# subramen/distributed-pytorch

Hardware: AMD Instinct MI355X
Metric: samples/sec (whole node), toy Linear DDP (higher is better)
Workload: dtype fp32; 1 GPU; model=Linear(20,1), global_batch=32, in_features=20, dataset_size=2048, parallelism=dp1, comm=none, engine=persistent, loss=mse, epoch_block=16

## Files before the change

mi355x_ddp/ops/csrc/toy_kernels.hip:

```cpp

#include <hip/hip_runtime.h>

#include <atomic>
#include <cstdint>
#include <cstdlib>
#include <string>
#include <type_traits>

#include "kernel_common.h"
#include "ops.h"
#include "p2p_mesh.h"

namespace mi355x {


__device__ __forceinline__ bool toy_mfma_db(int K) { return (K & 15) != 0; }

__device__ __forceinline__ float toy_db_wave_sum(const float* dy_s, int B,
                                                 int lane) {
  float dbp = 0.f;
  for (int i = lane; i < B; i += 64) dbp += dy_s[i];
  return wave_sum(dbp);
}

template <int MT, int KT>
__device__ __forceinline__ float toy_tile_step(
    const float* xs, const float* ts, const float* ws, float* dy_s,
    float bterm, bool mfma_db, int B, int K, int use_mse, int r, int q,
    f32x4 (&gacc)[KT]) {
  const float inv2B = 2.f / (float)B;
  float loss_acc = 0.f;
  {
    f32x4 acc[MT];
#pragma unroll
    for (int tm = 0; tm < MT; ++tm) acc[tm] = {0.f, 0.f, 0.f, 0.f};
    for (int k0 = 0; k0 < K; k0 += 4) {
      const int k = k0 + q;
      const float b = (r == 0 && k < K) ? ws[k] : 0.f;
#pragma unroll
      for (int tm = 0; tm < MT; ++tm) {
        const int m = tm * 16 + r;
        const float a = (m < B && k < K) ? xs[m * K + k] : 0.f;
        acc[tm] = __builtin_amdgcn_mfma_f32_16x16x4f32(a, b, acc[tm], 0, 0, 0);
      }
    }
#pragma unroll
    for (int tm = 0; tm < MT; ++tm) {
      if (r == 0) {
#pragma unroll
        for (int i = 0; i < 4; ++i) {
          const int row = tm * 16 + q * 4 + i;
          if (row < B) {
            const float y = acc[tm][i] + bterm;
            float dy;
            if (use_mse) {
              const float d = y - ts[row];
              loss_acc += d * d;
              dy = d * inv2B;
            } else {
              dy = 0.f;
            }
            dy_s[row] = dy;
          }
        }
      }
    }
  }
  __syncthreads();

#pragma unroll
  for (int tk = 0; tk < KT; ++tk) gacc[tk] = {0.f, 0.f, 0.f, 0.f};
  for (int i0 = 0; i0 < B; i0 += 4) {
    const int i = i0 + q;
    const float a = (r == 0 && i < B) ? dy_s[i] : 0.f;
#pragma unroll
    for (int tk = 0; tk < KT; ++tk) {
      const int k = tk * 16 + r;
      const float b = (i < B && k < K) ? xs[i * K + k]
                     : (i < B && k == K && mfma_db) ? 1.f : 0.f;
      gacc[tk] = __builtin_amdgcn_mfma_f32_16x16x4f32(a, b, gacc[tk], 0, 0, 0);
    }
  }
  return loss_acc;
}

template <typename T, int MT, int KT>
__global__ void k_toy_fused(const T* __restrict__ X, const T* __restrict__ Tg,
                            T* __restrict__ param, T* __restrict__ grad,
                            float* __restrict__ loss_out,
                            int B, int K, int use_mse,
                            int w_off, int b_off, float lr) {
  const int lane = threadIdx.x;
  const int r = lane & 15, q = lane >> 4;
  __shared__ float xs[128 * 32];
  __shared__ float ts[128];
  __shared__ float ws[33];
  __shared__ float dy_s[128];

  {
    const int total = B * K;
    for (int i = lane; i < total; i += 64) xs[i] = ldf(&X[i]);
    for (int i = lane; i < B; i += 64) ts[i] = ldf(&Tg[i]);
    if (lane < K) ws[lane] = ldf(&param[w_off + lane]);
    if (lane == K) ws[32] = ldf(&param[b_off]);
  }
  __syncthreads();

  const float bterm = ws[32];
  const bool mfma_db = toy_mfma_db(K);
  f32x4 acc[KT];
  float loss_acc = toy_tile_step<MT, KT>(xs, ts, ws, dy_s, bterm, mfma_db, B,
                                         K, use_mse, r, q, acc);
#pragma unroll
  for (int tk = 0; tk < KT; ++tk) {
    const int k = tk * 16 + r;
    if (q == 0 && k < K) {
      if (lr > 0.f) stf(&param[w_off + k], ws[k] - lr * acc[tk][0]);
      else stf(&grad[w_off + k], acc[tk][0]);
    } else if (q == 0 && k == K && mfma_db) {
      if (lr > 0.f) stf(&param[b_off], bterm - lr * acc[tk][0]);
      else stf(&grad[b_off], acc[tk][0]);
    }
  }
  if (!mfma_db) {
    const float dbp = toy_db_wave_sum(dy_s, B, lane);
    if (lane == 0) {
      if (lr > 0.f) stf(&param[b_off], bterm - lr * dbp);
      else stf(&grad[b_off], dbp);
    }
  }
  if (use_mse && loss_out) loss_acc = wave_sum(loss_acc);
  if (lane == 0 && loss_out) *loss_out = use_mse ? loss_acc / (float)B : 0.f;
}

template <typename T>
__device__ __forceinline__ float round_store(float v);
template <>
__device__ __forceinline__ float round_store<float>(float v) { return v; }
template <>
__device__ __forceinline__ float round_store<__hip_bfloat16>(float v) {
  return __bfloat162float(__float2bfloat16(v));
}

template <typename T, int MT, int KT>
__global__ void k_toy_multistep(const T* __restrict__ X,
                                const T* __restrict__ Tg,
                                T* __restrict__ param,
                                float* __restrict__ loss_out,
                                int B, int K, int S, int use_mse,
                                int w_off, int b_off, float lr) {
  constexpr int NR = (MT * 16 * KT * 16 + 63) / 64;
  constexpr int NT = (MT * 16 + 63) / 64;
  const int lane = threadIdx.x;
  const int r = lane & 15, q = lane >> 4;
  __shared__ float xs2[2][128 * 32];
  __shared__ float ts2[2][128];
  __shared__ float ws[33];
  __shared__ float dy_s[128];

  if (lane < K) ws[lane] = ldf(&param[w_off + lane]);
  if (lane == K) ws[32] = ldf(&param[b_off]);

  const int total = B * K;
  float xr[NR], tr[NT];
#pragma unroll
  for (int j = 0; j < NR; ++j) {
    const int i = lane + j * 64;
    if (i < total) xr[j] = ldf(&X[i]);
  }
#pragma unroll
  for (int j = 0; j < NT; ++j) {
    const int i = lane + j * 64;
    if (i < B) tr[j] = ldf(&Tg[i]);
  }

  float loss_last = 0.f;
  for (int s = 0; s < S; ++s) {
    const int buf = s & 1;
    float* xs = xs2[buf];
    float* ts = ts2[buf];
#pragma unroll
    for (int j = 0; j < NR; ++j) {
      const int i = lane + j * 64;
      if (i < total) xs[i] = xr[j];
    }
#pragma unroll
    for (int j = 0; j < NT; ++j) {
      const int i = lane + j * 64;
      if (i < B) ts[i] = tr[j];
    }
    __syncthreads();
    if (s + 1 < S) {
      const T* Xn = X + (size_t)(s + 1) * total;
      const T* Tn = Tg + (size_t)(s + 1) * B;
#pragma unroll
      for (int j = 0; j < NR; ++j) {
        const int i = lane + j * 64;
        if (i < total) xr[j] = ldf(&Xn[i]);
      }
#pragma unroll
      for (int j = 0; j < NT; ++j) {
        const int i = lane + j * 64;
        if (i < B) tr[j] = ldf(&Tn[i]);
      }
    }

    const float bterm = ws[32];
    const bool mfma_db = toy_mfma_db(K);
    f32x4 acc[KT];
    const float loss_acc = toy_tile_step<MT, KT>(
        xs, ts, ws, dy_s, bterm, mfma_db, B, K, use_mse, r, q, acc);
    __syncthreads();
#pragma unroll
    for (int tk = 0; tk < KT; ++tk) {
      const int k = tk * 16 + r;
      if (q == 0 && k < K)
        ws[k] = round_store<T>(ws[k] - lr * acc[tk][0]);
      else if (q == 0 && k == K && mfma_db)
        ws[32] = round_store<T>(bterm - lr * acc[tk][0]);
    }
    if (!mfma_db) {
      const float dbp = toy_db_wave_sum(dy_s, B, lane);
      if (lane == 0) ws[32] = round_store<T>(bterm - lr * dbp);
    }
    if (use_mse && loss_out && s == S - 1) loss_last = wave_sum(loss_acc);
    __syncthreads();
  }

  if (lane < K) stf(&param[w_off + lane], ws[lane]);
  if (lane == K) stf(&param[b_off], ws[32]);
  if (lane == 0 && loss_out) *loss_out = use_mse ? loss_last / (float)B : 0.f;
}

struct MeshArgs {
  MeshSlot* const* peer_slots = nullptr;
  MeshSlot* my_mb = nullptr;
  int world = 1;
  float inv_world = 1.f;
  unsigned long long seq0 = 0;
  unsigned int* err = nullptr;
};

template <int KT>
__device__ __forceinline__ bool mesh_exchange(float (&gval)[KT], int K_,
                                              int lane, int r, int q,
                                              const MeshArgs& m, int s) {
  const unsigned long long sq = m.seq0 + (unsigned long long)s;
  if (q == 0) {
#pragma unroll
    for (int tk = 0; tk < KT; ++tk) {
      const int k = tk * 16 + r;
      if (k <= K_) {
        for (int p = 0; p < m.world; ++p) m.peer_slots[p]->data[k] = gval[tk];
      }
    }
  }
  __threadfence_system();
  __syncthreads();
  if (lane == 0) {
    for (int p = 0; p < m.world; ++p)
      __hip_atomic_store(&m.peer_slots[p]->seq, sq, __ATOMIC_RELEASE,
                         __HIP_MEMORY_SCOPE_SYSTEM);
  }
  bool timed_out = false;
  if (lane < m.world) {
    const unsigned long long t0c = __builtin_amdgcn_s_memrealtime();
    while (__hip_atomic_load(&m.my_mb[lane].seq, __ATOMIC_ACQUIRE,
                             __HIP_MEMORY_SCOPE_SYSTEM) < sq) {
      if (__builtin_amdgcn_s_memrealtime() - t0c > 500000000ull) {
        timed_out = true;
        break;
      }
      __builtin_amdgcn_s_sleep(8);
    }
  }
  if (__any(timed_out)) return false;
  __threadfence_system();
  __syncthreads();
  if (q == 0) {
#pragma unroll
    for (int tk = 0; tk < KT; ++tk) {
      const int k = tk * 16 + r;
      if (k <= K_) {
        float sum = 0.f;
        for (int p = 0; p < m.world; ++p) sum += m.my_mb[p].data[k];
        gval[tk] = sum * m.inv_world;
      }
    }
  }
  return true;
}

template <int B_, int K_, bool MESH = false>
__global__ void __launch_bounds__(64, 1)
k_toy_multistep_spec(const float* __restrict__ X, const float* __restrict__ Tg,
                     float* __restrict__ param, float* __restrict__ loss_out,
                     int S, int use_mse, int w_off, int b_off, float lr,
                     MeshSlot* const* __restrict__ peer_slots,
                     MeshSlot* __restrict__ my_mb, int mworld,
                     float minv_world, unsigned long long seq0,
                     unsigned int* __restrict__ mesh_err) {
  static_assert(B_ % 16 == 0, "whole 16-row tiles: rows carry no guards");
  constexpr int MT = B_ / 16;
  constexpr int KT = (K_ + 15) / 16;
  constexpr int KS = (K_ + 3) / 4;
  constexpr int BS = B_ / 4;
  const int lane = threadIdx.x;
  const int r = lane & 15, q = lane >> 4;
  __shared__ float ws[33];
  __shared__ float dy_s[B_];

  if (lane < K_) ws[lane] = param[w_off + lane];
  if (lane == K_) ws[32] = param[b_off];
  const float inv2B = 2.f / (float)B_;
  float wreg[KT];
#pragma unroll
  for (int tk = 0; tk < KT; ++tk) {
    const int k = tk * 16 + r;
    wreg[tk] = (k < K_) ? param[w_off + ((k < K_) ? k : 0)] : 0.f;
  }

  float cfA[MT][KS];
  float cbB[KT][BS];
  float ctR[MT][4];

  auto prefetch = [&](int s) {
    const float* Xs = X + (size_t)s * (B_ * K_);
    const float* Ts = Tg + (size_t)s * B_;
#pragma unroll
    for (int tm = 0; tm < MT; ++tm) {
      const int m = tm * 16 + r;
#pragma unroll
      for (int kk = 0; kk < KS; ++kk) {
        const int k = 4 * kk + q;
        const int kc = (k < K_) ? k : K_ - 1;
        cfA[tm][kk] = Xs[m * K_ + kc];
      }
    }
#pragma unroll
    for (int tk = 0; tk < KT; ++tk) {
      const int k = tk * 16 + r;
      const int kc = (k < K_) ? k : K_ - 1;
#pragma unroll
      for (int ii = 0; ii < BS; ++ii) cbB[tk][ii] = Xs[(4 * ii + q) * K_ + kc];
    }
#pragma unroll
    for (int tm = 0; tm < MT; ++tm)
#pragma unroll
      for (int i = 0; i < 4; ++i) ctR[tm][i] = Ts[tm * 16 + q * 4 + i];
  };

  prefetch(0);
  float loss_last = 0.f;
  for (int s = 0; s < S; ++s) {
    float wv[KS];
#pragma unroll
    for (int kk = 0; kk < KS; ++kk) {
      const int k = 4 * kk + q;
      const float v = ws[(k < K_) ? k : K_ - 1];
      wv[kk] = (r == 0 && k < K_) ? v : 0.f;
    }
    const float bterm = ws[32];

    f32x4 acc[MT];
#pragma unroll
    for (int tm = 0; tm < MT; ++tm) acc[tm] = {0.f, 0.f, 0.f, 0.f};
#pragma unroll
    for (int kk = 0; kk < KS; ++kk)
#pragma unroll
      for (int tm = 0; tm < MT; ++tm)
        acc[tm] = __builtin_amdgcn_mfma_f32_16x16x4f32(cfA[tm][kk], wv[kk],
                                                       acc[tm], 0, 0, 0);

    float loss_acc = 0.f;
    if (r == 0) {
#pragma unroll
      for (int tm = 0; tm < MT; ++tm)
#pragma unroll
        for (int i = 0; i < 4; ++i) {
          float dy = 0.f;
          if (use_mse) {
            const float d = acc[tm][i] + bterm - ctR[tm][i];
            loss_acc = __builtin_fmaf(d, d, loss_acc);
            dy = d * inv2B;
          }
          dy_s[tm * 16 + q * 4 + i] = dy;
        }
    }
    __syncthreads();

    float av[BS];
#pragma unroll
    for (int ii = 0; ii < BS; ++ii) {
      const float v = dy_s[4 * ii + q];
      av[ii] = (r == 0) ? v : 0.f;
    }
    f32x4 gacc[KT];
#pragma unroll
    for (int tk = 0; tk < KT; ++tk) gacc[tk] = {0.f, 0.f, 0.f, 0.f};
    static_assert(K_ % 16 != 0, "free db column requires K_ % 16 != 0");
#pragma unroll
    for (int ii = 0; ii < BS; ++ii)
#pragma unroll
      for (int tk = 0; tk < KT; ++tk) {
        const int k = tk * 16 + r;
        const float bop = (k == K_) ? 1.f : cbB[tk][ii];
        gacc[tk] = __builtin_amdgcn_mfma_f32_16x16x4f32(av[ii], bop,
                                                        gacc[tk], 0, 0, 0);
      }

    if (s + 1 < S) prefetch(s + 1);

    if (use_mse && loss_out && s == S - 1) loss_last = wave_sum(loss_acc);

    if constexpr (MESH) {
      float gval[KT];
#pragma unroll
      for (int tk = 0; tk < KT; ++tk) gval[tk] = gacc[tk][0];
      const MeshArgs m{peer_slots, my_mb, mworld, minv_world, seq0, mesh_err};
      if (!mesh_exchange<KT>(gval, K_, lane, r, q, m, s)) {
        if (lane == 0) *mesh_err = 1u;
        return;
      }
#pragma unroll
      for (int tk = 0; tk < KT; ++tk) gacc[tk][0] = gval[tk];
    }

#pragma unroll
    for (int tk = 0; tk < KT; ++tk) {
      const int k = tk * 16 + r;
      if (q == 0 && k < K_) {
        wreg[tk] = wreg[tk] - lr * gacc[tk][0];
        ws[k] = wreg[tk];
      } else if (q == 0 && k == K_) {
        ws[32] = bterm - lr * gacc[tk][0];
      }
    }
    __syncthreads();
  }

  if (lane < K_) param[w_off + lane] = ws[lane];
  if (lane == K_) param[b_off] = ws[32];
  if (lane == 0 && loss_out) *loss_out = use_mse ? loss_last / (float)B_ : 0.f;
}

template <int B_, int K_, bool MESH = false>
__global__ void __launch_bounds__(64, 1)
k_toy_multistep_bf16w(const __hip_bfloat16* __restrict__ X,
                      const __hip_bfloat16* __restrict__ Tg,
                      __hip_bfloat16* __restrict__ param,
                      float* __restrict__ loss_out,
                      int S, int use_mse, int w_off, int b_off, float lr,
                      MeshSlot* const* __restrict__ peer_slots,
                      MeshSlot* __restrict__ my_mb, int mworld,
                      float minv_world, unsigned long long seq0,
                      unsigned int* __restrict__ mesh_err) {
  static_assert((B_ == 32 || B_ == 64) && K_ <= 32,
                "bf16 wide path: B in {32, 64}, K<=32");
  constexpr int MT = B_ / 16;
  constexpr int BT = B_ / 32;
  constexpr int KT = (K_ + 15) / 16;
  const int lane = threadIdx.x;
  const int r = lane & 15, q = lane >> 4;
  __shared__ float ws[33];
  __shared__ float dy_s[B_];

  if (lane < K_) ws[lane] = ldf(&param[w_off + lane]);
  if (lane == K_) ws[32] = ldf(&param[b_off]);
  const float inv2B = 2.f / (float)B_;
  float wreg[KT];
#pragma unroll
  for (int tk = 0; tk < KT; ++tk) {
    const int k = tk * 16 + r;
    wreg[tk] = (k < K_) ? ldf(&param[w_off + ((k < K_) ? k : 0)]) : 0.f;
  }

  struct BSet {
    bf16x8 fa[MT];
    bf16x8 bb[BT][KT];
    float tR[MT][4];
  };
  BSet setA, setB;

  auto prefetch = [&](BSet& R, int s) {
    const __hip_bfloat16* Xs = X + (size_t)s * (B_ * K_);
    const __hip_bfloat16* Ts = Tg + (size_t)s * B_;
#pragma unroll
    for (int tm = 0; tm < MT; ++tm) {
      const int m = tm * 16 + r;
#pragma unroll
      for (int j = 0; j < 8; ++j) {
        const int k = q * 8 + j;
        const int kc = (k < K_) ? k : K_ - 1;
        R.fa[tm][j] = *reinterpret_cast<const __bf16*>(&Xs[(size_t)m * K_ + kc]);
      }
    }
#pragma unroll
    for (int bt = 0; bt < BT; ++bt)
#pragma unroll
      for (int tk = 0; tk < KT; ++tk) {
        const int k = tk * 16 + r;
        const int kc = (k < K_) ? k : K_ - 1;
#pragma unroll
        for (int j = 0; j < 8; ++j) {
          const int i = bt * 32 + q * 8 + j;
          R.bb[bt][tk][j] =
              *reinterpret_cast<const __bf16*>(&Xs[(size_t)i * K_ + kc]);
        }
      }
#pragma unroll
    for (int tm = 0; tm < MT; ++tm)
#pragma unroll
      for (int i = 0; i < 4; ++i)
        R.tR[tm][i] = ldf(&Ts[tm * 16 + q * 4 + i]);
  };

  prefetch(setA, 0);
  if (S > 1) prefetch(setB, 1);
  float loss_last = 0.f;
  auto body = [&](BSet& R, int s) {
    const bf16x8* cfa = R.fa;
    const auto& cbb = R.bb;
    const auto& ctR = R.tR;
    bf16x8 b8{};
#pragma unroll
    for (int j = 0; j < 8; ++j) {
      const int k = q * 8 + j;
      const float v = ws[(k < K_) ? k : K_ - 1];
      b8[j] = (r == 0 && k < K_) ? (__bf16)v : (__bf16)0.f;
    }
    const float bterm = ws[32];

    f32x4 acc[MT];
#pragma unroll
    for (int tm = 0; tm < MT; ++tm) {
      acc[tm] = {0.f, 0.f, 0.f, 0.f};
      acc[tm] = __builtin_amdgcn_mfma_f32_16x16x32_bf16(cfa[tm], b8,
                                                        acc[tm], 0, 0, 0);
    }

    float loss_acc = 0.f;
    if (r == 0) {
#pragma unroll
      for (int tm = 0; tm < MT; ++tm)
#pragma unroll
        for (int i = 0; i < 4; ++i) {
          const int row = tm * 16 + q * 4 + i;
          float dy = 0.f;
          if (use_mse) {
            const float d = acc[tm][i] + bterm - ctR[tm][i];
            loss_acc += d * d;
            dy = d * inv2B;
          }
          dy_s[row] = dy;
        }
    }
    __syncthreads();

    bf16x8 a8[BT];
#pragma unroll
    for (int bt = 0; bt < BT; ++bt)
#pragma unroll
      for (int j = 0; j < 8; ++j) {
        const float v = dy_s[bt * 32 + q * 8 + j];
        a8[bt][j] = (r == 0) ? (__bf16)v : (__bf16)0.f;
      }
    f32x4 gacc[KT];
    static_assert(K_ % 16 != 0, "free db column requires K_ % 16 != 0");
#pragma unroll
    for (int tk = 0; tk < KT; ++tk) {
      gacc[tk] = {0.f, 0.f, 0.f, 0.f};
#pragma unroll
      for (int bt = 0; bt < BT; ++bt) {
        bf16x8 bb = cbb[bt][tk];
        if (tk * 16 + r == K_) {
#pragma unroll
          for (int j = 0; j < 8; ++j) bb[j] = (__bf16)1.f;
        }
        gacc[tk] = __builtin_amdgcn_mfma_f32_16x16x32_bf16(a8[bt], bb,
                                                           gacc[tk], 0, 0, 0);
      }
    }

    if (s + 2 < S) prefetch(R, s + 2);

    if (use_mse && loss_out && s == S - 1) loss_last = wave_sum(loss_acc);

    if constexpr (MESH) {
      float gval[KT];
#pragma unroll
      for (int tk = 0; tk < KT; ++tk) gval[tk] = gacc[tk][0];
      const MeshArgs m{peer_slots, my_mb, mworld, minv_world, seq0, mesh_err};
      if (!mesh_exchange<KT>(gval, K_, lane, r, q, m, s)) {
        if (lane == 0) *mesh_err = 1u;
        return false;
      }
#pragma unroll
      for (int tk = 0; tk < KT; ++tk) gacc[tk][0] = gval[tk];
    }

#pragma unroll
    for (int tk = 0; tk < KT; ++tk) {
      const int k = tk * 16 + r;
      if (q == 0 && k < K_) {
        wreg[tk] = round_store<__hip_bfloat16>(wreg[tk] - lr * gacc[tk][0]);
        ws[k] = wreg[tk];
      } else if (q == 0 && k == K_) {
        ws[32] = round_store<__hip_bfloat16>(bterm - lr * gacc[tk][0]);
      }
    }
    __syncthreads();
    return true;
  };

  int s = 0;
  for (; s + 2 <= S; s += 2) {
    if (!body(setA, s)) return;
    if (!body(setB, s + 1)) return;
  }
  if (s < S && !body(setA, s)) return;

  if (lane < K_) stf(&param[w_off + lane], ws[lane]);
  if (lane == K_) stf(&param[b_off], ws[32]);
  if (lane == 0 && loss_out) *loss_out = use_mse ? loss_last / (float)B_ : 0.f;
}


struct RowPair {
  float lo, hi;
};
__device__ __forceinline__ RowPair bcast_rows01(float v, float v2) {
  const auto r = __builtin_amdgcn_permlane16_swap(
      __float_as_uint(v), __float_as_uint(v2), false, false);
  return {__uint_as_float(r[0]), __uint_as_float(r[1])};
}
__device__ __forceinline__ RowPair bcast_rows01(float v) {
  return bcast_rows01(v, v);
}
__device__ __forceinline__ RowPair bcast_halves(float v, float v2) {
  const auto r = __builtin_amdgcn_permlane32_swap(
      __float_as_uint(v), __float_as_uint(v2), false, false);
  return {__uint_as_float(r[0]), __uint_as_float(r[1])};
}
__device__ __forceinline__ RowPair bcast_halves(float v) {
  return bcast_halves(v, v);
}

#define BC_DPP(n) " row_newbcast:" #n " row_mask:0xf bank_mask:0xf\n\t"
#define BC_FMAC(src, x, n) \
  "v_fmac_f32_dpp %[acc], %[" #src "], %[" #x "]" BC_DPP(n)
#define BC_FMAC4(src, p, n0, n1, n2, n3)                  \
  BC_FMAC(src, p##0, n0) BC_FMAC(src, p##1, n1)           \
  BC_FMAC(src, p##2, n2) BC_FMAC(src, p##3, n3)
#define BC_FMAC16(src, p)                                             \
  BC_FMAC4(src, p##0, 0, 1, 2, 3) BC_FMAC4(src, p##1, 4, 5, 6, 7)     \
  BC_FMAC4(src, p##2, 8, 9, 10, 11) BC_FMAC4(src, p##3, 12, 13, 14, 15)
#define BC_IN4(p, x)                                            \
  [p##0] "v"((x)[0]), [p##1] "v"((x)[1]), [p##2] "v"((x)[2]),   \
  [p##3] "v"((x)[3])
#define BC_IN16(p, x)                                     \
  BC_IN4(p##0, (x)) , BC_IN4(p##1, (x) + 4),              \
  BC_IN4(p##2, (x) + 8), BC_IN4(p##3, (x) + 12)
#define BC_PAD "s_nop 1\n\t"
#define BC_ZERO "v_mov_b32 %[acc], 0\n\ts_nop 0\n\t"


template <bool MSE>
__device__ __forceinline__ void chain_fwd20(const RowPair& w,
                                            const float (&x)[20], float t,
                                            float scale, float& d,
                                            float& dy) {
  float acc;
  if constexpr (MSE) {
    asm volatile(BC_ZERO BC_FMAC16(lo, a) BC_FMAC4(hi, b, 0, 1, 2, 3)
                 "v_add_f32_dpp %[acc], %[hi], %[acc]" BC_DPP(4)
                 "v_sub_f32 %[d], %[acc], %[t]\n\t"
                 "v_mul_f32 %[dy], %[c], %[d]"
                 : [acc] "=&v"(acc), [d] "=&v"(d), [dy] "=&v"(dy)
                 : [lo] "v"(w.lo), [hi] "v"(w.hi), BC_IN16(a, x),
                   BC_IN4(b, x + 16), [t] "v"(t), [c] "s"(scale)
                 : "memory");
  } else {
    asm volatile(BC_ZERO BC_FMAC16(lo, a) BC_FMAC4(hi, b, 0, 1, 2, 3)
                 "v_add_f32_dpp %[acc], %[hi], %[acc]" BC_DPP(4)
                 "v_sub_f32 %[d], %[acc], %[t]"
                 : [acc] "=&v"(acc), [d] "=&v"(d)
                 : [lo] "v"(w.lo), [hi] "v"(w.hi), BC_IN16(a, x),
                   BC_IN4(b, x + 16), [t] "v"(t)
                 : "memory");
    dy = 0.f;
  }
}
enum ChainLink { kStart, kPad, kPlain };
template <ChainLink LINK>
__device__ __forceinline__ void chain_bwd16(float& acc, float src,
                                            const float* x) {
  if constexpr (LINK == kStart)
    asm volatile(BC_ZERO BC_FMAC16(s, a)
                 : [acc] "=&v"(acc)
                 : [s] "v"(src), BC_IN16(a, x));
  else if constexpr (LINK == kPad)
    asm volatile(BC_PAD BC_FMAC16(s, a)
                 : [acc] "+v"(acc)
                 : [s] "v"(src), BC_IN16(a, x));
  else
    asm volatile(BC_FMAC16(s, a)
                 : [acc] "+v"(acc)
                 : [s] "v"(src), BC_IN16(a, x));
}
__device__ __forceinline__ void chain_bwd16_update(float& acc, float src,
                                                   const float* x, float& w,
                                                   float lr) {
  asm volatile(BC_FMAC16(s, a) "v_fma_f32 %[w], -%[lr], %[acc], %[w]"
               : [acc] "+v"(acc), [w] "+v"(w)
               : [s] "v"(src), BC_IN16(a, x), [lr] "s"(lr));
}
#undef BC_ZERO
#undef BC_PAD
#undef BC_IN16
#undef BC_IN4
#undef BC_FMAC16
#undef BC_FMAC4
#undef BC_FMAC
#undef BC_DPP

template <int B_, int K_>
struct ChainSlot {
  static constexpr int kPitch = B_ + 4;
  static constexpr int kRow = 0;
  static constexpr int kTr = B_ * K_;
  static constexpr int kOnes = kTr + K_ * kPitch;
  static constexpr int kTgt = kTr + (K_ + 1) * kPitch;
  static constexpr int kSize = kTgt + B_;
  static constexpr int kMaxH = (64 * 1024 / 4) / kSize / 2;
  static_assert(kSize % 4 == 0 && kTr % 4 == 0 && kPitch % 4 == 0 &&
                    K_ % 4 == 0 && B_ % 4 == 0,
                "every ds_read_b128 must be 16-byte aligned");
};

static constexpr int kChainTilesAhead = 4;

template <int B_, int K_, int NL>
__global__ void __launch_bounds__(64 * (1 + NL))
k_toy_multistep_chain(const float* __restrict__ X,
                      const float* __restrict__ Tg,
                      float* __restrict__ param, float* __restrict__ loss_out,
                      int S, int H, int use_mse, int w_off, int b_off,
                      float lr) {
  static_assert((B_ == 32 || B_ == 64) && K_ == 20 && NL >= 1 && NL <= 3,
                "chain path: B in {32, 64}, K = 20, one wave per SIMD");
  using L = ChainSlot<B_, K_>;
  __shared__ __attribute__((aligned(16))) float ring[2 * L::kMaxH * L::kSize];
  const int wave = __builtin_amdgcn_readfirstlane((int)(threadIdx.x >> 6));

  if (wave != 0) {
    constexpr int NT = 64 * NL;
    constexpr int NX = (B_ * K_ + NT - 1) / NT;
    constexpr bool kTail = (B_ * K_) % NT != 0;
    constexpr int R = kChainTilesAhead;
    const int lt = (int)threadIdx.x - 64;
    const int total = (S + H - 1) / H * H;
    float xv[R][NX], tv[R];

    auto load_tile = [&](float (&x)[NX], float& t, int tile) {
      const int tc = tile < S ? tile : S - 1;
      const float* xt = X + (size_t)tc * (B_ * K_);
#pragma unroll
      for (int i = 0; i < NX; ++i) {
        const int f = lt + i * NT;
        x[i] = xt[(kTail && i == NX - 1 && f >= B_ * K_) ? B_ * K_ - 1 : f];
      }
      t = Tg[(size_t)tc * B_ + (lt & (B_ - 1))];
    };
    auto write_tile = [&](const float (&x)[NX], float t, int slot) {
      float* sl = ring + slot * L::kSize;
#pragma unroll
      for (int i = 0; i < NX; ++i) {
        const int f = lt + i * NT;
        if (!kTail || i < NX - 1 || f < B_ * K_) {
          sl[L::kRow + f] = x[i];
          sl[L::kTr + (f % K_) * L::kPitch + f / K_] = x[i];
        }
      }
      if (lt < B_) sl[L::kTgt + lt] = t;
    };

#pragma unroll
    for (int r = 0; r < R; ++r) load_tile(xv[r], tv[r], r);
    if (lt < B_)
      for (int sl = 0; sl < 2 * H; ++sl) ring[sl * L::kSize + L::kOnes + lt] = 1.f;
    int slot = 0, togo = H;
    for (int t0 = 0; t0 < total; t0 += R) {
#pragma unroll
      for (int r = 0; r < R; ++r) {
        const int tile = t0 + r;
        if (tile < S) write_tile(xv[r], tv[r], slot);
        load_tile(xv[r], tv[r], tile + R);
        slot = (slot + 1 == 2 * H) ? 0 : slot + 1;
        if (--togo == 0) {
          togo = H;
          if (tile < total) __syncthreads();
        }
      }
    }
    return;
  }

  const int lane = threadIdx.x;
  const int mr = lane & (B_ - 1);
  const int cr = (lane <= K_) ? lane : (lane & 15);
  const float inv2B = 2.f / (float)B_;
  float wv = param[(lane < K_) ? w_off + lane : b_off];
  const float* rowp = ring + L::kRow + mr * K_;
  const float* colp = ring + L::kTr + cr * L::kPitch;
  const float* tgtp = ring + L::kTgt + mr;

  struct LSet {
    f32x4 xr[K_ / 4];
    f32x4 xc[B_ / 4];
    float t;
  };
  LSet setA, setB;

  auto fetch = [&](LSet& R, int o) {
#pragma unroll
    for (int j = 0; j < K_ / 4; ++j)
      R.xr[j] = *reinterpret_cast<const f32x4*>(rowp + o + 4 * j);
#pragma unroll
    for (int j = 0; j < B_ / 4; ++j)
      R.xc[j] = *reinterpret_cast<const f32x4*>(colp + o + 4 * j);
    R.t = tgtp[o];
  };
  auto settle = [&](LSet& R) {
    static_assert(K_ == 20, "five row reads");
    if constexpr (B_ == 64)
      asm volatile(""
                   : "+v"(R.xc[8]), "+v"(R.xc[9]), "+v"(R.xc[10]),
                     "+v"(R.xc[11]), "+v"(R.xc[12]), "+v"(R.xc[13]),
                     "+v"(R.xc[14]), "+v"(R.xc[15]));
    asm volatile(""
                 : "+v"(R.xr[0]), "+v"(R.xr[1]), "+v"(R.xr[2]), "+v"(R.xr[3]),
                   "+v"(R.xr[4]), "+v"(R.xc[0]), "+v"(R.xc[1]), "+v"(R.xc[2]),
                   "+v"(R.xc[3]), "+v"(R.xc[4]), "+v"(R.xc[5]), "+v"(R.xc[6]),
                   "+v"(R.xc[7]), "+v"(R.t)
                 :
                 : "memory");
  };

  struct CSet {
    float xr[K_];
    float xc[B_];
    float t;
  };
  float wa, wb;
  auto dup = [&] {
    wa = wv, wb = wv;
    asm volatile("" : "+v"(wa), "+v"(wb)::"memory");
  };
  float d_last = 0.f;
  auto compute = [&](const LSet& V, auto mse) {
    CSet R;
#pragma unroll
    for (int k = 0; k < K_; ++k) R.xr[k] = V.xr[k / 4][k % 4];
#pragma unroll
    for (int i = 0; i < B_; ++i) R.xc[i] = V.xc[i / 4][i % 4];
    R.t = V.t;
    RowPair w;
    if constexpr (B_ == 64) w = bcast_rows01(bcast_halves(wa, wb).lo);
    else w = bcast_rows01(wa, wb);
    float d, dy;
    chain_fwd20<decltype(mse)::value>(w, R.xr, R.t, inv2B, d, dy);
    d_last = d;

    float g;
    if constexpr (B_ == 64) {
      const RowPair h = bcast_halves(dy);
      const RowPair p01 = bcast_rows01(h.lo), p23 = bcast_rows01(h.hi);
      chain_bwd16<kStart>(g, p01.lo, R.xc);
      chain_bwd16<kPlain>(g, p01.hi, R.xc + 16);
      chain_bwd16<kPad>(g, p23.lo, R.xc + 32);
      chain_bwd16_update(g, p23.hi, R.xc + 48, wv, lr);
    } else {
      const RowPair p = bcast_rows01(dy);
      chain_bwd16<kStart>(g, p.lo, R.xc);
      chain_bwd16_update(g, p.hi, R.xc + 16, wv, lr);
    }
    __builtin_amdgcn_wave_barrier();
  };

  int slot = 0;
  int togo = 0;
  const int slots = 2 * H;
  auto fetch_step = [&](LSet& R, int s) {
    if (s < S) {
      if (togo == 0) {
        __syncthreads();
        togo = H;
      }
      --togo;
      fetch(R, slot * L::kSize);
      slot = (slot + 1 == slots) ? 0 : slot + 1;
    }
  };
  asm volatile("" : "+v"(wv));
  fetch_step(setA, 0);
  int s = 0;

  auto turns = [&](auto hc) {
    constexpr int HC = decltype(hc)::value;
    for (; s + 2 * HC < S; s += 2 * HC) {
#pragma unroll
      for (int p = 0; p < HC; ++p) {
        constexpr int kTurn = 2 * HC;
        settle(setA);
        if ((2 * p + 1) % HC == 0) __syncthreads();
        dup();
        fetch(setB, (2 * p + 1) * L::kSize);
        compute(setA, std::true_type{});
        settle(setB);
        if ((2 * p + 2) % HC == 0) __syncthreads();
        dup();
        fetch(setA, (2 * p + 2) % kTurn * L::kSize);
        compute(setB, std::true_type{});
      }
    }
  };
  auto steps = [&](auto mse) {
    for (; s < S; s += 2) {
      settle(setA);
      dup();
      fetch_step(setB, s + 1);
      compute(setA, mse);
      if (s + 1 < S) {
        settle(setB);
        dup();
        fetch_step(setA, s + 2);
        compute(setB, mse);
      }
    }
  };
  if (use_mse) {
    if (H == 2) turns(std::integral_constant<int, 2>{});
    if constexpr (L::kMaxH >= 4) {
      if (H == 3) turns(std::integral_constant<int, 3>{});
      if (H == 4) turns(std::integral_constant<int, 4>{});
    }
    steps(std::true_type{});
  } else {
    steps(std::false_type{});
  }

  if (lane < K_) param[w_off + lane] = wv;
  if (lane == K_) param[b_off] = wv;
  if (loss_out) {
    float loss_last = 0.f;
    if (use_mse) {
      const int r = lane & 15, q = lane >> 4;
      float loss_acc = 0.f;
#pragma unroll
      for (int tm = 0; tm < B_ / 16; ++tm)
#pragma unroll
        for (int i = 0; i < 4; ++i) {
          const float dd = __shfl(d_last, tm * 16 + q * 4 + i, 64);
          if (r == 0) loss_acc = __builtin_fmaf(dd, dd, loss_acc);
        }
      loss_last = wave_sum(loss_acc);
    }
    if (lane == 0) *loss_out = use_mse ? loss_last / (float)B_ : 0.f;
  }
}

enum : int { kImplChain = 0, kImplMfma = 1 };
static int impl_from_env() {
  const char* e = std::getenv("MI355X_TOY_MULTISTEP");
  if (e == nullptr || *e == '\0' || std::string(e) == "chain") return kImplChain;
  TORCH_CHECK(std::string(e) == "mfma",
              "MI355X_TOY_MULTISTEP must be 'chain' or 'mfma', got '", e, "'");
  return kImplMfma;
}
static std::atomic<int>& multistep_impl() {
  static std::atomic<int> impl{impl_from_env()};
  return impl;
}
static std::atomic<int> g_chain_depth{0};

void set_toy_multistep_impl(const std::string& name) {
  TORCH_CHECK(name == "chain" || name == "mfma",
              "toy multistep impl must be 'chain' or 'mfma', got '", name, "'");
  multistep_impl().store(name == "chain" ? kImplChain : kImplMfma);
}
std::string get_toy_multistep_impl() {
  return multistep_impl().load() == kImplChain ? "chain" : "mfma";
}
void set_toy_multistep_chain_depth(int64_t depth) {
  TORCH_CHECK(depth == 0 || (depth >= 2 && depth <= 4),
              "chain ring depth (steps per ring half) must be 0 (default), "
              "2, 3 or 4");
  g_chain_depth.store((int)depth);
}

static constexpr int kChainDefaultH = 2;
static constexpr int kChainLoaderWaves32 = 2;
static constexpr int kChainLoaderWaves64 = 2;

template <int B_>
static void launch_toy_multistep_chain(const float* xp, const float* tp,
                                       float* pp, float* lossp, bool use_mse,
                                       int w_off, int b_off, float lr, int S) {
  constexpr int kMaxH = ChainSlot<B_, 20>::kMaxH;
  static_assert(kMaxH >= 2, "the ring needs two steps per half");
  int H = g_chain_depth.load();
  if (H == 0) H = kChainDefaultH;
  if (H > kMaxH) H = kMaxH;
  constexpr int NL = B_ == 64 ? kChainLoaderWaves64 : kChainLoaderWaves32;
  hipLaunchKernelGGL((k_toy_multistep_chain<B_, 20, NL>), dim3(1),
                     dim3(64 * (1 + NL)), 0, cur_stream(), xp, tp, pp, lossp,
                     S, H, use_mse ? 1 : 0, w_off, b_off, lr);
}

template <typename F>
static void with_fast_batch(int B, F&& fn) {
  if (B == 32) fn(std::integral_constant<int, 32>{});
  else fn(std::integral_constant<int, 64>{});
}

template <typename T, int B_, bool MESH>
static void launch_toy_multistep_mfma(const T* xp, const T* tp, T* pp,
                                      float* lossp, bool use_mse, int w_off,
                                      int b_off, float lr, int S,
                                      const MeshArgs& m = {}) {
  auto kptr = [] {
    if constexpr (std::is_same<T, __hip_bfloat16>::value)
      return &k_toy_multistep_bf16w<B_, 20, MESH>;
    else
      return &k_toy_multistep_spec<B_, 20, MESH>;
  }();
  hipLaunchKernelGGL(kptr, dim3(1), dim3(64), 0, cur_stream(), xp, tp, pp,
                     lossp, S, use_mse ? 1 : 0, w_off, b_off, lr, m.peer_slots,
                     m.my_mb, m.world, m.inv_world, m.seq0, m.err);
}

template <typename F>
static void with_toy_tiles(int B, int K, F&& fn) {
  using c1 = std::integral_constant<int, 1>;
  using c2 = std::integral_constant<int, 2>;
  using c4 = std::integral_constant<int, 4>;
  using c8 = std::integral_constant<int, 8>;
  const int mt = (B + 15) / 16, kt = (K + 15) / 16;
  auto by_mt = [&](auto ktc) {
    if (mt <= 1) fn(c1{}, ktc);
    else if (mt <= 2) fn(c2{}, ktc);
    else if (mt <= 4) fn(c4{}, ktc);
    else fn(c8{}, ktc);
  };
  if (kt <= 1) by_mt(c1{});
  else by_mt(c2{});
}

static float* loss_ptr(const torch::Tensor& loss_out) {
  if (!loss_out.defined() || !loss_out.numel()) return nullptr;
  TORCH_CHECK(loss_out.scalar_type() == at::kFloat, "loss_out must be f32");
  return loss_out.data_ptr<float>();
}

ToyDims toy_check_args(const char* who, const torch::Tensor& x,
                       const torch::Tensor& t, const torch::Tensor& param,
                       const torch::Tensor* grad, bool need_grad,
                       const torch::Tensor& loss_out, int64_t w_off,
                       int64_t b_off, int64_t batch) {
  TORCH_CHECK(x.defined() && t.defined() && param.defined(), who,
              ": x, t and param_flat must be tensors");
  TORCH_CHECK(x.is_cuda(), who, ": x must be on a GPU");
  const auto dev = x.device();
  const auto dt = x.scalar_type();
  TORCH_CHECK(dt == at::kFloat || dt == at::kBFloat16, who,
              ": dtype must be f32 or bf16, got ", dt);
  TORCH_CHECK(x.dim() == 2 && x.is_contiguous(), who,
              ": x must be [rows, K] and contiguous");
  const int64_t rows = x.size(0), K = x.size(1);
  TORCH_CHECK(t.device() == dev && t.scalar_type() == dt && t.is_contiguous() &&
                  t.numel() == rows,
              who, ": t must be contiguous, one target per row of x, with "
              "x's dtype and device");
  TORCH_CHECK(K >= 1 && K <= 32, who, " supports 1 <= K <= 32, got K = ", K);
  if (batch < 0) batch = rows > 0 ? rows : 1;
  TORCH_CHECK(batch >= 1 && batch <= 128, who,
              " supports 1 <= batch <= 128, got batch = ", batch);
  TORCH_CHECK(rows % batch == 0 && rows / batch <= INT32_MAX, who,
              ": x rows must be a multiple of batch");
  auto check_bucket = [&](const torch::Tensor& b, const char* name) {
    TORCH_CHECK(b.device() == dev && b.scalar_type() == dt &&
                    b.is_contiguous(),
                who, ": ", name, " must be contiguous with x's dtype and device");
    const int64_t n = b.numel();
    TORCH_CHECK(n <= INT32_MAX && w_off >= 0 && b_off >= 0 &&
                    w_off + K <= n && b_off < n,
                who, ": w_off/b_off with K = ", K, " fall outside ", name,
                " (", n, " elements)");
    TORCH_CHECK(b_off < w_off || b_off >= w_off + K, who,
                ": b_off lies inside the weights [w_off, w_off + K)");
  };
  check_bucket(param, "param_flat");
  if (grad != nullptr) {
    const bool given = grad->defined() && grad->numel() > 0;
    TORCH_CHECK(given || !need_grad, who,
                ": lr <= 0 writes the gradients: grad_flat is required");
    if (given) check_bucket(*grad, "grad_flat");
  }
  if (loss_out.defined() && loss_out.numel() > 0)
    TORCH_CHECK(loss_out.device() == dev &&
                    loss_out.scalar_type() == at::kFloat,
                who, ": loss_out must be f32 on x's device");
  return {(int)batch, (int)K, (int)(rows / batch)};
}

template <typename T>
static void launch_toy_multistep(const T* xp, const T* tp, T* pp, float* lossp,
                                 bool use_mse, int w_off, int b_off, float lr,
                                 int B, int K, int S) {
  if ((B == 32 || B == 64) && K == 20) {
    with_fast_batch(B, [&](auto b) {
      constexpr int B_ = decltype(b)::value;
      if constexpr (std::is_same<T, float>::value) {
        if (multistep_impl().load() == kImplChain) {
          launch_toy_multistep_chain<B_>(xp, tp, pp, lossp, use_mse, w_off,
                                         b_off, lr, S);
          return;
        }
      }
      launch_toy_multistep_mfma<T, B_, false>(xp, tp, pp, lossp, use_mse,
                                              w_off, b_off, lr, S);
    });
    return;
  }
  with_toy_tiles(B, K, [&](auto mt, auto kt) {
    hipLaunchKernelGGL((k_toy_multistep<T, decltype(mt)::value, decltype(kt)::value>),
                       dim3(1), dim3(64), 0, cur_stream(), xp, tp, pp, lossp,
                       B, K, S, use_mse ? 1 : 0, w_off, b_off, lr);
  });
}

void toy_multistep_launch(const void* x, const void* t, void* param,
                          float* loss, bool use_mse, int w_off, int b_off,
                          float lr, int B, int K, int S, bool bf16) {
  if (bf16) {
    using T = __hip_bfloat16;
    launch_toy_multistep<T>(static_cast<const T*>(x), static_cast<const T*>(t),
                            static_cast<T*>(param), loss, use_mse, w_off,
                            b_off, lr, B, K, S);
  } else {
    launch_toy_multistep<float>(static_cast<const float*>(x),
                                static_cast<const float*>(t),
                                static_cast<float*>(param), loss, use_mse,
                                w_off, b_off, lr, B, K, S);
  }
  HIP_OK(hipGetLastError());
}

float* toy_loss_ptr(const torch::Tensor& loss_out) { return loss_ptr(loss_out); }

void toy_multistep(torch::Tensor x, torch::Tensor t, torch::Tensor param_flat,
                   torch::Tensor loss_out, bool use_mse,
                   int64_t w_off, int64_t b_off, double lr, int64_t batch) {
  TORCH_CHECK(batch >= 1, "toy_multistep: batch must be >= 1");
  const ToyDims d = toy_check_args("toy_multistep", x, t, param_flat, nullptr,
                                   false, loss_out, w_off, b_off, batch);
  TORCH_CHECK((float)lr > 0.f,
              "toy_multistep is the world-1 in-kernel-SGD path: lr must be > 0");
  if (d.S == 0) return;
  toy_multistep_launch(x.data_ptr(), t.data_ptr(), param_flat.data_ptr(),
                       loss_ptr(loss_out), use_mse, (int)w_off, (int)b_off,
                       (float)lr, d.B, d.K, d.S,
                       x.scalar_type() == at::kBFloat16);
}

void toy_multistep_mesh(torch::Tensor x, torch::Tensor t,
                        torch::Tensor param_flat, torch::Tensor loss_out,
                        bool use_mse, int64_t w_off, int64_t b_off, double lr,
                        int64_t batch, P2pMesh& mesh) {
  TORCH_CHECK(batch >= 1, "toy_multistep_mesh: batch must be >= 1");
  const ToyDims d = toy_check_args("toy_multistep_mesh", x, t, param_flat,
                                   nullptr, false, loss_out, w_off, b_off,
                                   batch);
  const int B = d.B, S = d.S;
  TORCH_CHECK((B == 32 || B == 64) && d.K == 20,
              "mesh multistep supports the fast-path shapes "
              "(batch 32 or 64, K 20)");
  TORCH_CHECK((float)lr > 0.f,
              "mesh multistep applies SGD in-kernel: lr must be > 0");
  TORCH_CHECK(mesh.connected(),
              "toy_multistep_mesh: the mesh is not connected");
  if (S == 0) return;
  float* lossp = loss_ptr(loss_out);
  const MeshArgs m{mesh.peer_slots(), mesh.my_mb(), mesh.world(),
                   1.f / (float)mesh.world(),
                   mesh.alloc_seq((unsigned long long)S), mesh.err_flag()};
  auto go = [&](auto zero) {
    using T = decltype(zero);
    with_fast_batch(B, [&](auto b) {
      launch_toy_multistep_mfma<T, decltype(b)::value, true>(
          cdptr<T>(x), cdptr<T>(t), dptr<T>(param_flat), lossp, use_mse,
          (int)w_off, (int)b_off, (float)lr, S, m);
    });
  };
  if (x.scalar_type() == at::kFloat) go(float{});
  else go(__hip_bfloat16{});
  HIP_OK(hipGetLastError());
}

template <typename T>
static void launch_toy_fused(const torch::Tensor& x, const torch::Tensor& t,
                             torch::Tensor& param_flat, torch::Tensor& grad_flat,
                             float* lossp, bool use_mse, int w_off, int b_off,
                             float lr, int B, int K) {
  const T* xp = cdptr<T>(x);
  const T* tp = cdptr<T>(t);
  T* pp = dptr<T>(param_flat);
  T* gp = grad_flat.defined() && grad_flat.numel() ? dptr<T>(grad_flat)
                                                   : nullptr;
  with_toy_tiles(B, K, [&](auto mt, auto kt) {
    hipLaunchKernelGGL((k_toy_fused<T, decltype(mt)::value, decltype(kt)::value>),
                       dim3(1), dim3(64), 0, cur_stream(), xp, tp, pp, gp,
                       lossp, B, K, use_mse ? 1 : 0, w_off, b_off, lr);
  });
}

void toy_fused_fwd_bwd(torch::Tensor x, torch::Tensor t,
                       torch::Tensor param_flat, torch::Tensor grad_flat,
                       torch::Tensor loss_out, bool use_mse,
                       int64_t w_off, int64_t b_off, double lr) {
  const ToyDims d = toy_check_args("toy_fused_fwd_bwd", x, t, param_flat,
                                   &grad_flat, !((float)lr > 0.f), loss_out,
                                   w_off, b_off, -1);
  if (d.S == 0) return;
  const int B = d.B, K = d.K;
  float* lossp = loss_ptr(loss_out);
  DISPATCH_F32_BF16(x.scalar_type(), "toy_fused_fwd_bwd", {
    launch_toy_fused<scalar_t>(x, t, param_flat, grad_flat, lossp, use_mse,
                               (int)w_off, (int)b_off, (float)lr, B, K);
  });
  HIP_OK(hipGetLastError());
}

}
```

Before: 158.7 million samples/s.

## Place chain loader waves on chosen SIMDs with LDS-conflict-aware element mapping

The chain kernel now always launches four waves, with a bitmask picking which waves act as loaders (waves 1 and 3). Idle waves only take part in the barriers. Loader threads use a row/column grouped mapping so that global loads and the transposed LDS writes cover each element exactly once with fewer bank conflicts. A sched_barrier is added between prefetch tiles, and the default ring depth rises from 2 to 3 steps per half. The intent is to spread loader waves across SIMDs away from the compute wave and cut LDS store conflicts. The cost is extra idle waves that still join every barrier, plus more index arithmetic per load.

```diff
diff --git a/mi355x_ddp/ops/csrc/toy_kernels.hip b/mi355x_ddp/ops/csrc/toy_kernels.hip
--- a/mi355x_ddp/ops/csrc/toy_kernels.hip
+++ b/mi355x_ddp/ops/csrc/toy_kernels.hip
@@ -740,25 +740,50 @@
 
 static constexpr int kChainTilesAhead = 4;
 
-template <int B_, int K_, int NL>
-__global__ void __launch_bounds__(64 * (1 + NL))
+static constexpr int kChainWaves = 4;
+template <int B_, int K_, unsigned LMASK>
+__global__ void __launch_bounds__(64 * kChainWaves)
 k_toy_multistep_chain(const float* __restrict__ X,
                       const float* __restrict__ Tg,
                       float* __restrict__ param, float* __restrict__ loss_out,
                       int S, int H, int use_mse, int w_off, int b_off,
                       float lr) {
-  static_assert((B_ == 32 || B_ == 64) && K_ == 20 && NL >= 1 && NL <= 3,
-                "chain path: B in {32, 64}, K = 20, one wave per SIMD");
+  constexpr int NL = __builtin_popcount(LMASK);
+  constexpr int G = 2 * NL;
+  static_assert((B_ == 32 || B_ == 64) && K_ == 20 && (LMASK & 1u) == 0 &&
+                    LMASK < (1u << kChainWaves) && (NL == 1 || NL == 2),
+                "chain path: B in {32, 64}, K = 20, wave 0 computes, one or "
+                "two of waves 1..3 load");
+  static_assert((B_ / 4) % G == 0 && (B_ / 8) % G == 0,
+                "the loader groups tile the rows exactly");
   using L = ChainSlot<B_, K_>;
   __shared__ __attribute__((aligned(16))) float ring[2 * L::kMaxH * L::kSize];
   const int wave = __builtin_amdgcn_readfirstlane((int)(threadIdx.x >> 6));
 
+  if (wave != 0 && !((LMASK >> wave) & 1u)) {
+    const int NC = (S + H - 1) / H;
+    for (int c = 0; c < NC; ++c) __syncthreads();
+    return;
+  }
   if (wave != 0) {
-    constexpr int NT = 64 * NL;
-    constexpr int NX = (B_ * K_ + NT - 1) / NT;
-    constexpr bool kTail = (B_ * K_) % NT != 0;
+    constexpr int RPI = B_ / 4 / G;
+    constexpr int NXA = 2 * RPI, NXB = B_ / 8 / G, NX = NXA + NXB;
+    static_assert(NX * 64 * NL == B_ * K_, "every element exactly once");
     constexpr int R = kChainTilesAhead;
-    const int lt = (int)threadIdx.x - 64;
+    const int lt = 64 * __builtin_popcount(LMASK & ((1u << wave) - 1u)) +
+                   (int)(threadIdx.x & 63);
+    const int g = lt >> 5, l = lt & 31;
+    const int rowA = 4 * g + (l >> 3), kA = l & 7;
+    const int rowB = 8 * g + (l >> 2), kB = 16 + (l & 3);
+    auto row_off = [&](int i) {
+      return i < NXA ? (rowA + 4 * G * (i % RPI)) * K_ + kA + 8 * (i / RPI)
+                     : (rowB + 8 * G * (i - NXA)) * K_ + kB;
+    };
+    auto tr_off = [&](int i) {
+      return i < NXA
+                 ? (kA + 8 * (i / RPI)) * L::kPitch + rowA + 4 * G * (i % RPI)
+                 : kB * L::kPitch + rowB + 8 * G * (i - NXA);
+    };
     const int total = (S + H - 1) / H * H;
     float xv[R][NX], tv[R];
 
@@ -766,27 +791,24 @@
       const int tc = tile < S ? tile : S - 1;
       const float* xt = X + (size_t)tc * (B_ * K_);
 #pragma unroll
-      for (int i = 0; i < NX; ++i) {
-        const int f = lt + i * NT;
-        x[i] = xt[(kTail && i == NX - 1 && f >= B_ * K_) ? B_ * K_ - 1 : f];
-      }
+      for (int i = 0; i < NX; ++i) x[i] = xt[row_off(i)];
       t = Tg[(size_t)tc * B_ + (lt & (B_ - 1))];
     };
     auto write_tile = [&](const float (&x)[NX], float t, int slot) {
       float* sl = ring + slot * L::kSize;
 #pragma unroll
       for (int i = 0; i < NX; ++i) {
-        const int f = lt + i * NT;
-        if (!kTail || i < NX - 1 || f < B_ * K_) {
-          sl[L::kRow + f] = x[i];
-          sl[L::kTr + (f % K_) * L::kPitch + f / K_] = x[i];
-        }
+        sl[L::kRow + row_off(i)] = x[i];
+        sl[L::kTr + tr_off(i)] = x[i];
       }
       if (lt < B_) sl[L::kTgt + lt] = t;
     };
 
 #pragma unroll
-    for (int r = 0; r < R; ++r) load_tile(xv[r], tv[r], r);
+    for (int r = 0; r < R; ++r) {
+      load_tile(xv[r], tv[r], r);
+      __builtin_amdgcn_sched_barrier(0);
+    }
     if (lt < B_)
       for (int sl = 0; sl < 2 * H; ++sl) ring[sl * L::kSize + L::kOnes + lt] = 1.f;
     int slot = 0, togo = H;
@@ -999,9 +1021,9 @@
   g_chain_depth.store((int)depth);
 }
 
-static constexpr int kChainDefaultH = 2;
-static constexpr int kChainLoaderWaves32 = 2;
-static constexpr int kChainLoaderWaves64 = 2;
+static constexpr int kChainDefaultH = 3;
+static constexpr unsigned kChainLoaders32 = 0b1010;
+static constexpr unsigned kChainLoaders64 = 0b1010;
 
 template <int B_>
 static void launch_toy_multistep_chain(const float* xp, const float* tp,
@@ -1012,10 +1034,10 @@
   int H = g_chain_depth.load();
   if (H == 0) H = kChainDefaultH;
   if (H > kMaxH) H = kMaxH;
-  constexpr int NL = B_ == 64 ? kChainLoaderWaves64 : kChainLoaderWaves32;
-  hipLaunchKernelGGL((k_toy_multistep_chain<B_, 20, NL>), dim3(1),
-                     dim3(64 * (1 + NL)), 0, cur_stream(), xp, tp, pp, lossp,
-                     S, H, use_mse ? 1 : 0, w_off, b_off, lr);
+  constexpr unsigned LM = B_ == 64 ? kChainLoaders64 : kChainLoaders32;
+  hipLaunchKernelGGL((k_toy_multistep_chain<B_, 20, LM>), dim3(1),
+                     dim3(64 * kChainWaves), 0, cur_stream(), xp, tp, pp,
+                     lossp, S, H, use_mse ? 1 : 0, w_off, b_off, lr);
 }
 
 template <typename F>
```

After: 167.7 million samples/s (median of 6 runs). +5.7%, better.
